# caburu/gym-supplychain

Measured on AMD Instinct MI355X. Metric: env-steps/sec at 65536 envs/GPU, beergame-v0; 1/2/4/8 MI355X, higher is better.
Workload: dtype int32; 1 GPU; beergame-v0 step() x 65536 envs/GPU (BASELINE configs[1]; configs[4] at N=8); n_envs_per_gpu=65536, levels=4, weeks=35, auto_reset=True, ledgers=True, orders_history=True, episode_return_allgather=False, parallelism=env-shard x1

## Files before the change

gym-supplychain_amd/csrc/scg_beergame.hip:

```cpp

#include <cstdarg>
#include <cstdio>
#include <ctime>
#include <vector>

#include "scg_beergame_kernels.h"

namespace scg {

__global__ __launch_bounds__(kBlock) void poisson_demand_kernel(const BgArgs a, int32_t weeks,
                                                                int32_t* __restrict__ out) {
  const int64_t n = static_cast<int64_t>(blockIdx.x) * kBlock + threadIdx.x;
  if (n >= a.n) return;
  for (int32_t w = 1; w <= weeks; ++w) out[(int64_t)(w - 1) * a.n + n] = week_demand(a, n, w, a.episode);
}

__global__ __launch_bounds__(kBlock) void uniform_ints_kernel(uint32_t k0, uint32_t k1, int64_t env_offset,
                                                              int64_t n_envs, int32_t rows, int32_t width,
                                                              uint32_t tag, int32_t lo, uint32_t range,
                                                              int32_t* __restrict__ out) {
  const int64_t n = static_cast<int64_t>(blockIdx.x) * kBlock + threadIdx.x;
  if (n >= n_envs) return;
  const uint32_t env = static_cast<uint32_t>(env_offset + n);
  const int32_t words = rows * width;
  for (int32_t j0 = 0; j0 < words; j0 += 4) {
    const scg::U4 r = scg::philox4x32_10(scg::U4{env, tag, static_cast<uint32_t>(j0 >> 2), SCG_STREAM_ACTION}, k0, k1);
    const uint32_t w4[4] = {r.x, r.y, r.z, r.w};
#pragma unroll
    for (int s = 0; s < 4; ++s) {
      const int32_t j = j0 + s;
      if (j < words) {
        const uint32_t v = static_cast<uint32_t>((static_cast<uint64_t>(w4[s]) * range) >> 32);
        const int32_t rrow = j / width, col = j - rrow * width;
        out[((int64_t)rrow * n_envs + n) * width + col] = lo + static_cast<int32_t>(v);
      }
    }
  }
}

int launch_reset(int L, dim3 grid, hipStream_t s, const BgArgs& a) {
  switch (L) {
#define X(l) case l: return bg_launch_reset<l>(grid, s, a);
    SCG_LEVEL_CASES(X)
#undef X
    default: return fail(SCG_ERR_INVALID, "levels=%d outside 1..%d", L, SCG_BG_MAX_LEVELS);
  }
}

int launch_step2(int L, dim3 grid, hipStream_t s, const BgArgs& a, const WeekInfo& wk) {
  switch (L) {
#define X(l) case l: return bg_launch_step2<l>(grid, s, a, wk);
    SCG_LEVEL_CASES(X)
#undef X
    default: return fail(SCG_ERR_INVALID, "levels=%d outside 1..%d", L, SCG_BG_MAX_LEVELS);
// ... 8 lines not shown
#undef X
    default: return fail(SCG_ERR_INVALID, "levels=%d outside 1..%d", L, SCG_BG_MAX_LEVELS);
  }
}

int launch_server(int L, int demand_mode, hipStream_t s, scg_bg_server_box* box, uint32_t exit_seen,
                  uint32_t idle_ticks) {
  switch (L) {
#define X(l) case l: return bg_launch_server<l>(s, demand_mode, box, exit_seen, idle_ticks);
    SCG_LEVEL_CASES(X)
#undef X
    default: return fail(SCG_ERR_INVALID, "levels=%d outside 1..%d", L, SCG_BG_MAX_LEVELS);
  }
}

int launch_slab(int demand_mode, int L, dim3 grid, hipStream_t s, int32_t* slab, const int32_t* act, int32_t* out,
                uint32_t n32, uint32_t wpack, uint32_t week, uint32_t episode, uint32_t k0, uint32_t k1,
                const BgSlabArgs& a, hipEvent_t ev0, hipEvent_t ev1) {
  switch (L) {
#define X(l) case l: return bg_launch_slab<l>(demand_mode, grid, s, slab, act, out, n32, wpack, week, episode, k0, k1, a, ev0, ev1);
    SCG_LEVEL_CASES(X)
#undef X
    default: return fail(SCG_ERR_INVALID, "levels=%d outside 1..%d", L, SCG_BG_MAX_LEVELS);
  }
}

int launch_rollout(int L, dim3 grid, hipStream_t s, const BgArgs& a, int32_t K, const RolloutWeeks& weeks,
                   const int32_t* acts, int32_t* obs, int32_t* rew) {
  switch (L) {
#define X(l) case l: return bg_launch_rollout<l>(grid, s, a, K, weeks, acts, obs, rew);
    SCG_LEVEL_CASES(X)
#undef X
    default: return fail(SCG_ERR_INVALID, "levels=%d outside 1..%d", L, SCG_BG_MAX_LEVELS);
  }
}
// ... 2 lines not shown
  const int64_t NL = N * L;
  if (NL % 4 != 0) return fail(SCG_ERR_INVALID, "slab layout needs n_envs * levels %% 4 == 0 (got %lld)", (long long)NL);
  if (R < 1 || R > 127) return fail(SCG_ERR_INVALID, "slab layout needs 1 <= ring_slots <= 127");
  off[SCG_SLAB_ERROR] = 0;
  for (int f = 0; f < 6; ++f) off[SCG_SLAB_INVENTORY + f] = kSlabHeader + f * NL;
  off[SCG_SLAB_RING] = kSlabHeader + 6 * NL;
  off[SCG_SLAB_EPISODE_RETURN] = kSlabHeader + (6 + R) * NL;
  off[SCG_SLAB_FINAL_RETURN] = off[SCG_SLAB_EPISODE_RETURN] + 2 * N;
  off[SCG_SLAB_HISTORY] = off[SCG_SLAB_FINAL_RETURN] + 2 * N;
  off[SCG_SLAB_TOTAL] = off[SCG_SLAB_HISTORY] + (history ? static_cast<int64_t>(T + 1) * NL : 0);
  return SCG_OK;
}

bool slab_ready(const scg_bg_config* cfg, const scg_bg_state* st, const int32_t* obs, const int32_t* reward,
                const int32_t* terminal_obs) {
  if (!st->slab || cfg->variant != 1) return false;
  int64_t off[SCG_SLAB_FIELDS];
  const bool hist = st->orders_history != nullptr;
  if (slab_layout(cfg->levels, st->n_envs, cfg->ring_slots, cfg->max_weeks, hist, off) != SCG_OK) return false;
  int32_t* b = st->slab;
  const bool ledgers = st->inventory_costs != nullptr, returns = st->episode_return != nullptr;
  return st->inventory == b + off[SCG_SLAB_INVENTORY] && st->backlog == b + off[SCG_SLAB_BACKLOG] &&
         st->orders_placed == b + off[SCG_SLAB_ORDERS] && st->shipments == b + off[SCG_SLAB_RING] &&
         (!ledgers || (st->inventory_costs == b + off[SCG_SLAB_INV_COSTS] &&
                       st->backlog_costs == b + off[SCG_SLAB_BACKLOG_COSTS])) &&
         ledgers == (st->backlog_costs != nullptr) &&
         (!returns || (reinterpret_cast<int32_t*>(st->episode_return) == b + off[SCG_SLAB_EPISODE_RETURN] &&
                       reinterpret_cast<int32_t*>(st->final_return) == b + off[SCG_SLAB_FINAL_RETURN])) &&
         (!hist || st->orders_history == b + off[SCG_SLAB_HISTORY]) &&
         st->error_flags == b + off[SCG_SLAB_ERROR] && reward == obs + st->n_envs * cfg->levels &&
         (!terminal_obs || terminal_obs == b + off[SCG_SLAB_TERMINAL_OBS]);
// ... 55 lines not shown
  a.guard = week_guard(cfg->levels, cfg->inv_cost, cfg->backlog_cost);
  a.err_host = st->error_host;
  if (cfg->variant == 2) {
    a.pen_acc = st->penalty_costs;
    a.max_stock = cfg->max_stock;
    a.penalty = cfg->exceeded_capacity_penalty;
    a.stochastic_delays = cfg->stochastic_delays;
    a.delay_lo = cfg->delay_lo;
    a.delay_hi = cfg->delay_hi;
  }
  return a;
}

inline dim3 grid_for(int64_t n) { return dim3(static_cast<unsigned>((n + kBlock - 1) / kBlock)); }

}

using namespace scg;

extern "C" {

int scg_bg_struct_sizes(size_t* config_size, size_t* state_size) {
  if (config_size) *config_size = sizeof(scg_bg_config);
  if (state_size) *state_size = sizeof(scg_bg_state);
  return SCG_OK;
}

int scg_poisson_table(double lam, uint32_t* out, int32_t cap) {
  if (!(lam >= 0.0) || std::isinf(lam)) return -fail(SCG_ERR_INVALID, "poisson lambda must be finite and >= 0");
  if (!out || cap <= 0) return -fail(SCG_ERR_INVALID, "null/empty threshold buffer");
// ... 112 lines not shown

int scg_bg_step(const scg_bg_config* cfg, scg_bg_state* st, const int32_t* action, int32_t* obs,
                int32_t* reward, int32_t* terminal_obs, uint32_t flags, int32_t* done, void* stream) {
  return scg_bg_step_timed(cfg, st, action, obs, reward, terminal_obs, flags, done, nullptr, nullptr, stream);
}

int scg_bg_step_timed(const scg_bg_config* cfg, scg_bg_state* st, const int32_t* action, int32_t* obs,
                      int32_t* reward, int32_t* terminal_obs, uint32_t flags, int32_t* done, void* start_event,
                      void* stop_event, void* stream) {
  if (int rc = check_state(cfg, st)) return rc;
  if (!action || !obs || !reward) return fail(SCG_ERR_INVALID, "action/obs/reward buffers are required");
  if (int rc = check_step(cfg, st)) return rc;
  const int32_t w = st->week + 1;
  const WeekInfo wk = week_info(cfg, w, flags);
  if (slab_ready(cfg, st, obs, reward, terminal_obs)) {
    BgSlabArgs sa;
    std::memset(&sa, 0, sizeof(sa));
    sa.pthr = cfg->poisson_thresholds;
    sa.demand_table = cfg->demand_table;
    sa.pthr_len = cfg->poisson_len;
    sa.h = cfg->inv_cost;
    sa.b = cfg->backlog_cost;
    sa.demand_fixed = wk.demand_fixed;
    sa.demand_lo = cfg->demand_lo;
    sa.demand_hi = cfg->demand_hi;
    sa.ship_value = cfg->initial_shipment_value;
    sa.orders_value = cfg->initial_orders_value;
    sa.init_slots = init_slots(cfg);
    sa.env_offset = st->env_offset;
    sa.guard = week_guard(cfg->levels, cfg->inv_cost, cfg->backlog_cost);
    sa.err_host = st->error_host;
    for (int l = 0; l < cfg->levels; ++l) sa.init_inv[l] = cfg->initial_inventory[l];
    uint32_t wpack = pack_week_slab(wk);
    wpack |= (wk.flags & 1) ? SW_TERMINAL : 0u;
    wpack |= (wk.flags & 2) ? SW_AUTORESET : 0u;
    wpack |= st->inventory_costs ? SW_LEDGERS : 0u;
    wpack |= st->episode_return ? SW_RETURNS : 0u;
    wpack |= st->orders_history ? SW_HISTORY : 0u;
    wpack |= static_cast<uint32_t>(cfg->ring_slots) << 24;
    if (int rc = launch_slab(cfg->demand_mode, cfg->levels, grid_for(st->n_envs), static_cast<hipStream_t>(stream),
                             st->slab, action, obs, static_cast<uint32_t>(st->n_envs), wpack, static_cast<uint32_t>(w),
                             st->episode, static_cast<uint32_t>(st->seed & 0xffffffffu),
                             static_cast<uint32_t>(st->seed >> 32), sa, static_cast<hipEvent_t>(start_event),
                             static_cast<hipEvent_t>(stop_event)))
      return rc;
    if (wk.flags & 2) {
      st->week = 0;
      st->episode += 1;
    } else {
      st->week = w;
    }
    if (done) *done = (wk.flags & 1) ? 1 : 0;
    return SCG_OK;
  }
  BgArgs a = make_args(cfg, st);
  a.act = action;
  a.obs = obs;
  a.rew = reward;
  a.term_obs = terminal_obs;
// ... 280 lines not shown
```

gym-supplychain_amd/csrc/scg_beergame_kernels.h:

```cpp
#pragma once

#include <hip/hip_ext.h>
#include <hip/hip_runtime.h>

#include <algorithm>
#include <cmath>
#include <cstdint>
#include <cstdlib>
#include <cstring>

#include "scg_common.h"
#include "scg_mailbox.h"
#include "scg_const.h"
#include "scg_philox.h"
#include "scgpu.h"

namespace scg {

enum : int32_t { MODE_DIRECT = 0, MODE_STORE = 1, MODE_ADD = 2, MODE_DROP = 3 };
constexpr int32_t PLAN_ARRIVE = 4;
inline int32_t plan_mode(int32_t p) { return p & 3; }
inline bool plan_arrive(int32_t p) { return (p & PLAN_ARRIVE) != 0; }
inline int32_t plan_delay(int32_t p) { return (p >> 8) & 0xff; }

// ... 79 lines not shown
    for (int c = 0; c < L / 4; ++c)
      reinterpret_cast<int4*>(p)[c] = make_int4(v[4 * c], v[4 * c + 1], v[4 * c + 2], v[4 * c + 3]);
  } else if constexpr (L % 2 == 0) {
#pragma unroll
    for (int c = 0; c < L / 2; ++c) reinterpret_cast<int2*>(p)[c] = make_int2(v[2 * c], v[2 * c + 1]);
  } else {
#pragma unroll
    for (int l = 0; l < L; ++l) p[l] = v[l];
  }
}

#ifndef SCG_BG_STORE
#define SCG_BG_STORE 1
#endif
typedef int v4i32 __attribute__((ext_vector_type(4)));

template <int L>
__device__ __forceinline__ void store_row_p(int32_t* __restrict__ p, const int32_t (&v)[L]) {
  if constexpr (SCG_BG_STORE != 0 && L % 4 == 0) {
#pragma unroll
    for (int c = 0; c < L / 4; ++c) {
      const v4i32 x = {v[4 * c], v[4 * c + 1], v[4 * c + 2], v[4 * c + 3]};
      if constexpr (SCG_BG_STORE == 1) {
        __builtin_nontemporal_store(x, reinterpret_cast<v4i32*>(p) + c);
      } else {
        asm volatile("global_store_dwordx4 %0, %1, off sc1\n\ts_nop 1" ::"v"(reinterpret_cast<v4i32*>(p) + c), "v"(x)
                     : "memory");
      }
    }
  } else {
// ... 8 lines not shown
  for (int l = 0; l < L; ++l) v[l] = x;
  store_row_p<L>(p, v);
}

template <int L>
__device__ __forceinline__ void fill_row(int32_t* __restrict__ p, int32_t x) {
  int32_t v[L];
#pragma unroll
  for (int l = 0; l < L; ++l) v[l] = x;
  store_row<L>(p, v);
}

__device__ __forceinline__ int32_t poisson_count_scalar(ConstTab<uint32_t> thr, int32_t len, uint32_t u) {
  int32_t x = 0;
  int k = 0;
  for (; k + 8 <= len; k += 8) {
#pragma unroll
    for (int j = 0; j < 8; ++j) x += (thr[k + j] <= u) ? 1 : 0;
  }
  for (; k < len; ++k) x += (thr[k] <= u) ? 1 : 0;
  return x;
}

__device__ __forceinline__ int32_t poisson_invert(const BgArgs& a, uint32_t u) {
  return poisson_count_scalar(const_tab(a.pthr), a.pthr_len, u);
}

template <int DM = -1>
__device__ __forceinline__ int32_t week_demand(const BgArgs& a, int64_t n, int32_t week,
                                               uint32_t episode) {
// ... 371 lines not shown
      __syncthreads();
      served = true;
    }
    if (ex != exit_seen) break;
    if (served) {
      t0 = __builtin_amdgcn_s_memrealtime();
      continue;
    }
    if (__builtin_amdgcn_s_memrealtime() - t0 > idle_ticks) break;
    __builtin_amdgcn_s_sleep(2);
  }
  __builtin_amdgcn_fence(__ATOMIC_RELEASE, "");
  if (lane == 0) __hip_atomic_store(&box->exit_seq, ex, __ATOMIC_RELEASE, __HIP_MEMORY_SCOPE_SYSTEM);
}

struct BgSlabArgs {
  const uint32_t* pthr;
  const int32_t* demand_table;
  int32_t pthr_len;
  int32_t h, b;
  int32_t demand_fixed;
  int32_t demand_lo, demand_hi;
  int32_t ship_value, orders_value, init_slots;
  int64_t env_offset;
  int32_t guard;
  int32_t* err_host;
  int32_t init_inv[SCG_BG_MAX_LEVELS];
};


constexpr uint32_t SW_TERMINAL = 1u << 18, SW_AUTORESET = 1u << 19, SW_LEDGERS = 1u << 20, SW_RETURNS = 1u << 21,
                   SW_HISTORY = 1u << 22;
constexpr int kSlabHeader = 4;

template <int L, int DM>
__global__ __launch_bounds__(kBlock) void bg_step_slab_kernel(int32_t* __restrict__ slab, const int32_t* __restrict__ act_p,
                                                              int32_t* __restrict__ out, uint32_t n32, uint32_t wpack,
                                                              uint32_t week, uint32_t episode, uint32_t key0,
                                                              uint32_t key1, const BgSlabArgs a) {
  const int64_t n = static_cast<int64_t>(blockIdx.x) * kBlock + threadIdx.x;
  if (n >= static_cast<int64_t>(n32)) return;
  const int32_t read_slot = static_cast<int32_t>(wpack & 0xffu) - 1;
  const int32_t write_slot = static_cast<int32_t>((wpack >> 8) & 0xffu);
  const int32_t mode = static_cast<int32_t>((wpack >> 16) & 3u);
  const int32_t R = static_cast<int32_t>((wpack >> 24) & 0x7fu);
  const bool terminal = wpack & SW_TERMINAL, autoreset = wpack & SW_AUTORESET;
  const bool ledgers = wpack & SW_LEDGERS, returns = wpack & SW_RETURNS, history = wpack & SW_HISTORY;
  const int64_t NL = static_cast<int64_t>(n32) * L;
  const int64_t row = n * L;
  int32_t* const rows = slab + kSlabHeader;
  int32_t* const inv_p = rows, *const bk_p = rows + NL, *const op_p = rows + 2 * NL;
  int32_t* const iacc_p = rows + 3 * NL, *const bacc_p = rows + 4 * NL, *const term_p = rows + 5 * NL;
  int32_t* const ring_p = rows + 6 * NL;
  int64_t* const ret_p = reinterpret_cast<int64_t*>(rows + (6 + R) * NL);
  int64_t* const fret_p = ret_p + n32;
  int32_t* const hist_p = reinterpret_cast<int32_t*>(fret_p + n32);
// ... 2 lines not shown
  zero_row<L>(due);
  zero_row<L>(cur);
  zero_row<L>(iacc);
  zero_row<L>(bacc);
  load_row<L>(inv_p + row, inv);
  load_row<L>(bk_p + row, bk);
  load_row<L>(op_p + row, op);
  load_row<L>(act_p + row, act);
  if (read_slot >= 0) load_row<L>(ring_p + read_slot * NL + row, due);
  if (mode == MODE_ADD) load_row<L>(ring_p + write_slot * NL + row, cur);
  if (ledgers && !autoreset) {
    load_row<L>(iacc_p + row, iacc);
    load_row<L>(bacc_p + row, bacc);
  }
  const int64_t ret0 = returns ? ret_p[n] : 0;
  export_error(n, terminal, slab, a.err_host);
  int32_t demand;
  if constexpr (DM == SCG_DEMAND_FIXED) {
    demand = a.demand_fixed;
  } else if constexpr (DM == SCG_DEMAND_TABLE) {
    demand = a.demand_table[static_cast<int64_t>(week - 1) * n32 + n];
  } else if constexpr (DM == SCG_DEMAND_UNIFORM) {
    const uint32_t w = scg::philox_word(key0, key1, static_cast<uint32_t>(a.env_offset + n), episode, week - 1,
                                        SCG_STREAM_BG2_DEMAND);
    demand = a.demand_lo + static_cast<int32_t>((static_cast<uint64_t>(w) * static_cast<uint32_t>(a.demand_hi - a.demand_lo)) >> 32);
  } else {
    const uint32_t u = scg::philox_word(key0, key1, static_cast<uint32_t>(a.env_offset + n), episode, week - 1,
                                        SCG_STREAM_DEMAND);
    demand = poisson_count_scalar(const_tab(a.pthr), a.pthr_len, u);
  }

  int32_t ship[L], obs[L];
  bool ovf = false;
  const int32_t reward = week_update<L>(a.h, a.b, a.guard, demand, mode == MODE_DIRECT, due, inv, bk, op, act, ship,
                                        obs, cur, iacc, bacc, ovf);
  if (mode == MODE_STORE) {
    store_row_p<L>(ring_p + write_slot * NL + row, ship);
  } else if (mode == MODE_ADD) {
    store_row_p<L>(ring_p + write_slot * NL + row, cur);
  }
  out[NL + n] = reward;
  if (history) store_row_p<L>(hist_p + static_cast<int64_t>(week) * NL + row, op);
  const int64_t ret = ret0 + reward;
  if (terminal) {
    store_row_p<L>(term_p + row, obs);
    if (returns) fret_p[n] = ret;
  }
  if (autoreset) {
    int32_t v[L];
#pragma unroll
    for (int l = 0; l < L; ++l) v[l] = a.init_inv[l];
    store_row_p<L>(inv_p + row, v);
    store_row_p<L>(out + row, v);
    fill_row_p<L>(bk_p + row, 0);
    fill_row_p<L>(op_p + row, a.orders_value);
    for (int t = 1; t <= a.init_slots; ++t) fill_row_p<L>(ring_p + (t % R) * NL + row, a.ship_value);
    if (ledgers) {
      fill_row_p<L>(iacc_p + row, 0);
      fill_row_p<L>(bacc_p + row, 0);
    }
    if (history) fill_row_p<L>(hist_p + row, a.orders_value);
    if (returns) ret_p[n] = 0;
    note_overflow(slab, ovf);
    return;
  }
  store_row_p<L>(inv_p + row, inv);
  store_row_p<L>(bk_p + row, bk);
  store_row_p<L>(op_p + row, op);
  store_row_p<L>(out + row, obs);
  if (ledgers) {
    store_row_p<L>(iacc_p + row, iacc);
    store_row_p<L>(bacc_p + row, bacc);
  }
  if (returns) ret_p[n] = ret;
  note_overflow(slab, ovf);
}
// ... 235 lines not shown
    hbm.load(s, v);
    lds.store(s, v);
  }
  rollout_body<L>(a, n, K, weeks, acts, obs_out, rew_out, lds);
  for (int s = 0; s < a.ring_slots; ++s) {
    int32_t v[L];
    lds.load(s, v);
    hbm.store(s, v);
  }
}

#ifndef SCG_MODULE_LAUNCH
#define SCG_MODULE_LAUNCH 1
#endif

template <int L, int DM>
int launch_slab_module(dim3 grid, hipStream_t s, int32_t* slab, const int32_t* act, int32_t* out, uint32_t n32,
                       uint32_t wpack, uint32_t week, uint32_t episode, uint32_t k0, uint32_t k1, const BgSlabArgs& a) {
  static hipFunction_t fn = nullptr;
  if (!fn && hipGetFuncBySymbol(&fn, reinterpret_cast<const void*>(&bg_step_slab_kernel<L, DM>)) != hipSuccess)
    return fail(SCG_ERR_HIP, "hipGetFuncBySymbol(bg_step_slab_kernel) failed");
  BgSlabArgs args = a;
  void* params[] = {&slab, &act, &out, &n32, &wpack, &week, &episode, &k0, &k1, &args};
  if (hipModuleLaunchKernel(fn, grid.x, 1, 1, kBlock, 1, 1, 0, s, params, nullptr) != hipSuccess)
    return fail(SCG_ERR_HIP, "hipModuleLaunchKernel(bg_step_slab_kernel) failed");
  return SCG_OK;
}

template <int L>
int bg_launch_reset(dim3 grid, hipStream_t s, const BgArgs& a) {
  hipLaunchKernelGGL(bg_reset_kernel<L>, grid, dim3(kBlock), 0, s, a);
  return check_launch("bg_reset_kernel");
}

template <int L>
int bg_launch_step2(dim3 grid, hipStream_t s, const BgArgs& a, const WeekInfo& wk) {
  hipLaunchKernelGGL(bg2_step_kernel<L>, grid, dim3(kBlock), 0, s, a, wk);
  return check_launch("bg2_step_kernel");
// ... 27 lines not shown
      hipLaunchKernelGGL(HIP_KERNEL_NAME(bg_server_kernel<L, SCG_DEMAND_TABLE>), dim3(1), dim3(kServerBlock), 0, s, box,
                         exit_seen, idle_ticks);
      break;
    case SCG_DEMAND_UNIFORM:
      hipLaunchKernelGGL(HIP_KERNEL_NAME(bg_server_kernel<L, SCG_DEMAND_UNIFORM>), dim3(1), dim3(kServerBlock), 0, s, box,
                         exit_seen, idle_ticks);
      break;
    default:
      hipLaunchKernelGGL(HIP_KERNEL_NAME(bg_server_kernel<L, SCG_DEMAND_POISSON>), dim3(1), dim3(kServerBlock), 0, s, box,
                         exit_seen, idle_ticks);
  }
  return check_launch("bg_server_kernel");
}

template <int L, int DM>
int bg_launch_slab_dm(dim3 grid, hipStream_t s, int32_t* slab, const int32_t* act, int32_t* out, uint32_t n32,
                      uint32_t wpack, uint32_t week, uint32_t episode, uint32_t k0, uint32_t k1, const BgSlabArgs& a,
                      hipEvent_t ev0, hipEvent_t ev1) {
  if (ev0 || ev1) {
    hipExtLaunchKernelGGL(HIP_KERNEL_NAME(bg_step_slab_kernel<L, DM>), grid, dim3(kBlock), 0, s, ev0, ev1, 0, slab, act,
                          out, n32, wpack, week, episode, k0, k1, a);
    return check_launch("bg_step_slab_kernel");
  }
  if (SCG_MODULE_LAUNCH) return launch_slab_module<L, DM>(grid, s, slab, act, out, n32, wpack, week, episode, k0, k1, a);
  hipLaunchKernelGGL(HIP_KERNEL_NAME(bg_step_slab_kernel<L, DM>), grid, dim3(kBlock), 0, s, slab, act, out, n32, wpack,
                     week, episode, k0, k1, a);
  return check_launch("bg_step_slab_kernel");
}

template <int L>
int bg_launch_slab(int demand_mode, dim3 grid, hipStream_t s, int32_t* slab, const int32_t* act, int32_t* out,
                   uint32_t n32, uint32_t wpack, uint32_t week, uint32_t episode, uint32_t k0, uint32_t k1,
                   const BgSlabArgs& a, hipEvent_t ev0, hipEvent_t ev1) {
  switch (demand_mode) {
    case SCG_DEMAND_FIXED:
      return bg_launch_slab_dm<L, SCG_DEMAND_FIXED>(grid, s, slab, act, out, n32, wpack, week, episode, k0, k1, a, ev0, ev1);
    case SCG_DEMAND_TABLE:
      return bg_launch_slab_dm<L, SCG_DEMAND_TABLE>(grid, s, slab, act, out, n32, wpack, week, episode, k0, k1, a, ev0, ev1);
    case SCG_DEMAND_UNIFORM:
      return bg_launch_slab_dm<L, SCG_DEMAND_UNIFORM>(grid, s, slab, act, out, n32, wpack, week, episode, k0, k1, a, ev0,
                                                      ev1);
    default:
      return bg_launch_slab_dm<L, SCG_DEMAND_POISSON>(grid, s, slab, act, out, n32, wpack, week, episode, k0, k1, a, ev0,
                                                      ev1);
  }
}

template <int L>
int bg_launch_rollout(dim3 grid, hipStream_t s, const BgArgs& a, int32_t K, const RolloutWeeks& weeks,
                      const int32_t* acts, int32_t* obs, int32_t* rew) {
  const size_t lds = static_cast<size_t>(a.ring_slots) * L * kBlock * sizeof(int32_t);
  if (lds <= 64 * 1024) {
    hipLaunchKernelGGL(bg_rollout_lds_kernel<L>, grid, dim3(kBlock), lds, s, a, K, weeks, acts, obs, rew);
    return check_launch("bg_rollout_lds_kernel");
  }
  hipLaunchKernelGGL(bg_rollout_kernel<L>, grid, dim3(kBlock), 0, s, a, K, weeks, acts, obs, rew);
  return check_launch("bg_rollout_kernel");
}

#define SCG_LEVEL_CASES(X) X(1) X(2) X(3) X(4) X(5) X(6) X(7) X(8) X(9) X(10) X(11) X(12) X(13) X(14) X(15) X(16)

#define SCG_BG_LAUNCHERS(EXT, l)                                                                                     \
  EXT template int bg_launch_reset<l>(dim3, hipStream_t, const BgArgs&);                                            \
  EXT template int bg_launch_step2<l>(dim3, hipStream_t, const BgArgs&, const WeekInfo&);                           \
  EXT template int bg_launch_step<l>(dim3, hipStream_t, const BgArgs&, const WeekInfo&, hipEvent_t, hipEvent_t);    \
  EXT template int bg_launch_server<l>(hipStream_t, int, scg_bg_server_box*, uint32_t, uint32_t);                   \
  EXT template int bg_launch_slab<l>(int, dim3, hipStream_t, int32_t*, const int32_t*, int32_t*, uint32_t, uint32_t, \
                                     uint32_t, uint32_t, uint32_t, uint32_t, const BgSlabArgs&, hipEvent_t,         \
                                     hipEvent_t);                                                                    \
  EXT template int bg_launch_rollout<l>(dim3, hipStream_t, const BgArgs&, int32_t, const RolloutWeeks&,             \
                                        const int32_t*, int32_t*, int32_t*);
#define SCG_BG_EXTERN_LEVEL(l) SCG_BG_LAUNCHERS(extern, l)
SCG_LEVEL_CASES(SCG_BG_EXTERN_LEVEL)
#undef SCG_BG_EXTERN_LEVEL

}
```

gym-supplychain_amd/gym_supplychain_amd/_native.py:

```python
import ctypes
import os

import torch

LIB_NAME = "libscgpu.so"
LIB_PATH = os.path.join(os.path.dirname(os.path.abspath(__file__)), LIB_NAME)
ABI_VERSION = 7

SCG_OK = 0
SCG_ERR_INVALID = 1
SCG_ERR_PAST_HORIZON = 2
SCG_ERR_NOT_RESET = 3
SCG_ERR_HIP = 4
SCG_PENDING = 5

SCG_DEMAND_FIXED = 0
SCG_DEMAND_TABLE = 1
SCG_DEMAND_POISSON = 2
SCG_DEMAND_UNIFORM = 3

SCG_BG_AUTORESET = 1
SCG_SC_SERIAL = 2
SCG_STREAM_DEMAND = 0
SCG_STREAM_ACTION = 1
# ... 48 lines not shown
        ("episode", ctypes.c_uint32),
        ("week", ctypes.c_int32),
        ("inventory", ctypes.c_void_p),
        ("backlog", ctypes.c_void_p),
        ("orders_placed", ctypes.c_void_p),
        ("shipments", ctypes.c_void_p),
        ("inventory_costs", ctypes.c_void_p),
        ("backlog_costs", ctypes.c_void_p),
        ("orders_history", ctypes.c_void_p),
        ("episode_return", ctypes.c_void_p),
        ("final_return", ctypes.c_void_p),
        ("penalty_costs", ctypes.c_void_p),
        ("error_flags", ctypes.c_void_p),
        ("error_host", ctypes.c_void_p),
        ("slab", ctypes.c_void_p),
    ]


BG_SERVER_SLOTS = 15
BG_SERVER_ARGS_BYTES = 512


class BgServerLine(ctypes.Structure):
    _fields_ = [("req_seq", ctypes.c_uint32), ("cmd", ctypes.c_int32), ("wpack", ctypes.c_uint32),
                ("week", ctypes.c_int32), ("demand_fixed", ctypes.c_int32), ("n_inline", ctypes.c_int32),
                ("gen", ctypes.c_uint32), ("check", ctypes.c_uint32), ("action", ctypes.c_int32 * 8)]


class BgServerBox(ctypes.Structure):
    _fields_ = [("req", BgServerLine * (BG_SERVER_SLOTS + 1)), ("done_seq", ctypes.c_uint32 * 16),
                ("n_slots", ctypes.c_uint32), ("exit_req", ctypes.c_uint32), ("exit_seq", ctypes.c_uint32),
# ... 347 lines not shown
```

gym-supplychain_amd/gym_supplychain_amd/envs/beergame_env.py:

```python
import atexit
import ctypes
import numbers
import os
import weakref

import numpy as np
import torch

from .. import _native as nat
from .. import checkpoint as ckpt
from .. import spaces
from . import resident
from ..distributed import entropy_seed

STD_LEVELS = 4
STD_DEMAND = [4] * 4 + [8] * 31
STD_INVENTORY = 12
STD_SHIP_DELAY = 2
STD_SHIP_VALUE = 4
STD_ORDERS_VALUE = 4
STD_INV_COST = 1
STD_BACKLOG_COST = 2

_I32 = (-(2 ** 31), 2 ** 31 - 1)
# ... 119 lines not shown
                raise ValueError(f"demand table must be int32 [{T}, {n_envs}] on {dev}")
            self._table = table.contiguous()
            c.demand_table = self._table.data_ptr()
        if mode == nat.SCG_DEMAND_POISSON:
            thr = nat.poisson_table(poisson_lambda)
            self.poisson_lambda = float(poisson_lambda)
            self._thresholds = torch.tensor(np.asarray(thr, dtype=np.uint32).view(np.int32), **i32)
            c.poisson_thresholds = self._thresholds.data_ptr()
            c.poisson_len = len(thr)
        nat.check(nat.lib.scg_bg_prepare(ctypes.byref(c)))
        self._cfg = c
        self.ring_slots = R = c.ring_slots

        v2 = c.variant == 2
        off = (ctypes.c_int64 * nat.SLAB_FIELDS)()
        self._slab = None
        if state_slab and nat.lib.scg_bg_slab_layout(ctypes.byref(c), n_envs, int(bool(track_history)), off) == 0:
            self._slab = torch.zeros(off[nat.SLAB_TOTAL], **i32)

            def rows(field, k=1):
                return self._slab[off[field]: off[field] + k * n_envs * L].view(*((k,) if k > 1 else ()), n_envs, L)

            def i64(field):
                return self._slab[off[field]: off[field] + 2 * n_envs].view(torch.int64)

            self._err = self._slab[off[nat.SLAB_ERROR]: off[nat.SLAB_ERROR] + 1]
            self._inv, self._bk, self._op = rows(nat.SLAB_INVENTORY), rows(nat.SLAB_BACKLOG), rows(nat.SLAB_ORDERS)
            self._ring = rows(nat.SLAB_RING, R) if R > 1 else rows(nat.SLAB_RING).unsqueeze(0)
            self._inv_costs = rows(nat.SLAB_INV_COSTS) if track_costs else None
            self._bk_costs = rows(nat.SLAB_BACKLOG_COSTS) if track_costs else None
            self._hist = rows(nat.SLAB_HISTORY, T + 1) if track_history else None
            self._ret = i64(nat.SLAB_EPISODE_RETURN) if track_returns else None
            self._final_ret = i64(nat.SLAB_FINAL_RETURN) if track_returns else None
# ... 20 lines not shown

        s = nat.BgState()
        s.n_envs, s.env_offset, s.seed = n_envs, int(env_offset), int(seed) & 0xFFFFFFFFFFFFFFFF
        s.episode, s.week = 0, -1
        s.inventory, s.backlog, s.orders_placed = self._inv.data_ptr(), self._bk.data_ptr(), self._op.data_ptr()
        s.shipments = self._ring.data_ptr()
        s.inventory_costs = self._inv_costs.data_ptr() if track_costs else None
        s.backlog_costs = self._bk_costs.data_ptr() if track_costs else None
        s.orders_history = self._hist.data_ptr() if track_history else None
        s.episode_return = self._ret.data_ptr() if track_returns else None
        s.final_return = self._final_ret.data_ptr() if track_returns else None
        s.penalty_costs = self._pen_costs.data_ptr() if self._pen_costs is not None else None
        s.error_flags = self._err.data_ptr()
        s.error_host = self._err_word.dev
        s.slab = self._slab.data_ptr() if self._slab is not None else None
        self._st = s
        self._cfg_ref = ctypes.byref(self._cfg)
        self._st_ref = ctypes.byref(self._st)
        self._done_flag = ctypes.c_int32(0)
        self._done_ref = ctypes.byref(self._done_flag)
        self._flags = nat.SCG_BG_AUTORESET if self.auto_reset else 0
        self._act_shape = (n_envs, L)
        self._obs_ptr, self._rew_ptr = self._obs.data_ptr(), self._rew.data_ptr()
        self._term_ptr = self._term_obs.data_ptr()
        self._cfg_addr, self._st_addr = ctypes.addressof(self._cfg), ctypes.addressof(self._st)
        self._fast_step, self._fast_step_timed = nat.fast.bg_step, nat.fast.bg_step_timed
        self._step_args = nat.BgStepArgs(self._cfg_addr, self._st_addr, self._obs_ptr, self._rew_ptr, self._term_ptr,
                                         self._flags)
        self._step_handle = ctypes.addressof(self._step_args)
        self._fast_step_h = nat.fast.bg_step_h
# ... 603 lines not shown
```

include/scgpu.h:

```cpp
#ifndef SCGPU_H
#define SCGPU_H

#include <stddef.h>
#include <stdint.h>

#ifdef __cplusplus
extern "C" {
#endif

#define SCG_ABI_VERSION 7

#if defined(__GNUC__)
#define SCG_API __attribute__((visibility("default")))
#else
#define SCG_API
#endif

#define SCG_BG_MAX_LEVELS 16
#define SCG_BG_MAX_WEEKS 4096
#define SCG_BG_MAX_DELAY 4096
#define SCG_POISSON_MAX 256
#define SCG_BG_ROLLOUT_MAX 128

typedef enum scg_status {
  SCG_OK = 0,
// ... 50 lines not shown
  uint32_t episode;
  int32_t week;
  int32_t* inventory;
  int32_t* backlog;
  int32_t* orders_placed;
  int32_t* shipments;
  int32_t* inventory_costs;
  int32_t* backlog_costs;
  int32_t* orders_history;
  int64_t* episode_return;
  int64_t* final_return;
  int32_t* penalty_costs;
  int32_t* error_flags;
  int32_t* error_host;
  int32_t* slab;
} scg_bg_state;

enum scg_bg_slab_field {
  SCG_SLAB_ERROR = 0,
  SCG_SLAB_INVENTORY,
  SCG_SLAB_BACKLOG,
  SCG_SLAB_ORDERS,
  SCG_SLAB_INV_COSTS,
  SCG_SLAB_BACKLOG_COSTS,
  SCG_SLAB_TERMINAL_OBS,
  SCG_SLAB_RING,
  SCG_SLAB_EPISODE_RETURN,
  SCG_SLAB_FINAL_RETURN,
  SCG_SLAB_HISTORY,
  SCG_SLAB_TOTAL,
  SCG_SLAB_FIELDS
// ... 271 lines not shown
```

Before: 13.22 billion env-steps/s.

## Move slab step constants into a device-resident block and shrink kernel arguments

The per-step constants (costs, guard, demand bounds, init values, pointers) move out of the by-value kernel argument struct into a 64-byte-aligned device buffer. A tiny kernel fills it only when a hash of the config changes. The step kernel now takes a small argument list and loads the constants with scalar loads. Poisson thresholds are also cached as a padded 40-entry table read as vector scalar loads. This cuts kernel argument marshalling and host packing per step, at the cost of an ABI change, an extra state field, and hash-based invalidation that could miss a change to the table contents behind the same pointer.

```diff
diff --git a/gym-supplychain_amd/csrc/scg_beergame.hip b/gym-supplychain_amd/csrc/scg_beergame.hip
--- a/gym-supplychain_amd/csrc/scg_beergame.hip
+++ b/gym-supplychain_amd/csrc/scg_beergame.hip
@@ -38,6 +38,26 @@
   }
 }
 
+__global__ __launch_bounds__(64) void bg_slab_consts_kernel(BgSlabConst* __restrict__ dst, const BgSlabConst v) {
+  const int q = threadIdx.x;
+  if (q < kFastThr) dst->thr[q] = (v.pthr && q < v.pthr_len) ? v.pthr[q] : 0xffffffffu;
+  if (q < SCG_BG_MAX_LEVELS) dst->init_inv[q] = v.init_inv[q];
+  if (q != 63) return;
+  dst->env_base = v.env_base;
+  dst->pthr_len = v.pthr_len;
+  dst->h = v.h;
+  dst->b = v.b;
+  dst->guard = v.guard;
+  dst->demand_lo = v.demand_lo;
+  dst->demand_hi = v.demand_hi;
+  dst->ship_value = v.ship_value;
+  dst->orders_value = v.orders_value;
+  dst->init_slots = v.init_slots;
+  dst->err_host = v.err_host;
+  dst->demand_table = v.demand_table;
+  dst->pthr = v.pthr;
+}
+
 int launch_reset(int L, dim3 grid, hipStream_t s, const BgArgs& a) {
   switch (L) {
 #define X(l) case l: return bg_launch_reset<l>(grid, s, a);
@@ -76,11 +96,10 @@
   }
 }
 
-int launch_slab(int demand_mode, int L, dim3 grid, hipStream_t s, int32_t* slab, const int32_t* act, int32_t* out,
-                uint32_t n32, uint32_t wpack, uint32_t week, uint32_t episode, uint32_t k0, uint32_t k1,
-                const BgSlabArgs& a, hipEvent_t ev0, hipEvent_t ev1) {
+int launch_slab(int demand_mode, int L, dim3 grid, hipStream_t s, const SlabLaunch& a, hipEvent_t ev0,
+                hipEvent_t ev1) {
   switch (L) {
-#define X(l) case l: return bg_launch_slab<l>(demand_mode, grid, s, slab, act, out, n32, wpack, week, episode, k0, k1, a, ev0, ev1);
+#define X(l) case l: return bg_launch_slab<l>(demand_mode, grid, s, a, ev0, ev1);
     SCG_LEVEL_CASES(X)
 #undef X
     default: return fail(SCG_ERR_INVALID, "levels=%d outside 1..%d", L, SCG_BG_MAX_LEVELS);
@@ -113,7 +132,7 @@
 
 bool slab_ready(const scg_bg_config* cfg, const scg_bg_state* st, const int32_t* obs, const int32_t* reward,
                 const int32_t* terminal_obs) {
-  if (!st->slab || cfg->variant != 1) return false;
+  if (!st->slab || !st->step_consts || cfg->variant != 1) return false;
   int64_t off[SCG_SLAB_FIELDS];
   const bool hist = st->orders_history != nullptr;
   if (slab_layout(cfg->levels, st->n_envs, cfg->ring_slots, cfg->max_weeks, hist, off) != SCG_OK) return false;
@@ -199,6 +218,50 @@
 
 inline dim3 grid_for(int64_t n) { return dim3(static_cast<unsigned>((n + kBlock - 1) / kBlock)); }
 
+BgSlabConst slab_consts(const scg_bg_config* cfg, const scg_bg_state* st) {
+  BgSlabConst v;
+  std::memset(&v, 0, sizeof(v));
+  v.env_base = static_cast<uint32_t>(st->env_offset);
+  v.pthr_len = cfg->demand_mode == SCG_DEMAND_POISSON ? cfg->poisson_len : 0;
+  v.h = cfg->inv_cost;
+  v.b = cfg->backlog_cost;
+  v.guard = week_guard(cfg->levels, cfg->inv_cost, cfg->backlog_cost);
+  v.demand_lo = cfg->demand_lo;
+  v.demand_hi = cfg->demand_hi;
+  v.ship_value = cfg->initial_shipment_value;
+  v.orders_value = cfg->initial_orders_value;
+  v.init_slots = init_slots(cfg);
+  v.err_host = st->error_host;
+  v.demand_table = cfg->demand_table;
+  v.pthr = cfg->demand_mode == SCG_DEMAND_POISSON ? cfg->poisson_thresholds : nullptr;
+  for (int l = 0; l < cfg->levels; ++l) v.init_inv[l] = cfg->initial_inventory[l];
+  return v;
+}
+
+uint64_t slab_consts_tag(const BgSlabConst& v, const void* block) {
+  static_assert(offsetof(BgSlabConst, thr) % 8 == 0, "hashed as 64-bit words");
+  uint64_t w[offsetof(BgSlabConst, thr) / 8];
+  std::memcpy(w, &v, sizeof(w));
+  uint64_t h = 0x9E3779B97F4A7C15ull ^ reinterpret_cast<uintptr_t>(block);
+  for (uint64_t x : w) {
+    h = (h ^ x) * 0xFF51AFD7ED558CCDull;
+    h ^= h >> 29;
+  }
+  return h | 1u;
+}
+
+int sync_slab_consts(const scg_bg_config* cfg, scg_bg_state* st, hipStream_t s) {
+  const BgSlabConst v = slab_consts(cfg, st);
+  const uint64_t tag = slab_consts_tag(v, st->step_consts);
+  if (tag == st->step_consts_tag) return SCG_OK;
+  if (reinterpret_cast<uintptr_t>(st->step_consts) % alignof(BgSlabConst) != 0)
+    return fail(SCG_ERR_INVALID, "step_consts must be %d-byte aligned", static_cast<int>(alignof(BgSlabConst)));
+  hipLaunchKernelGGL(bg_slab_consts_kernel, dim3(1), dim3(64), 0, s, static_cast<BgSlabConst*>(st->step_consts), v);
+  if (int rc = check_launch("bg_slab_consts_kernel")) return rc;
+  st->step_consts_tag = tag;
+  return SCG_OK;
+}
+
 }
 
 using namespace scg;
@@ -341,23 +404,7 @@
   const int32_t w = st->week + 1;
   const WeekInfo wk = week_info(cfg, w, flags);
   if (slab_ready(cfg, st, obs, reward, terminal_obs)) {
-    BgSlabArgs sa;
-    std::memset(&sa, 0, sizeof(sa));
-    sa.pthr = cfg->poisson_thresholds;
-    sa.demand_table = cfg->demand_table;
-    sa.pthr_len = cfg->poisson_len;
-    sa.h = cfg->inv_cost;
-    sa.b = cfg->backlog_cost;
-    sa.demand_fixed = wk.demand_fixed;
-    sa.demand_lo = cfg->demand_lo;
-    sa.demand_hi = cfg->demand_hi;
-    sa.ship_value = cfg->initial_shipment_value;
-    sa.orders_value = cfg->initial_orders_value;
-    sa.init_slots = init_slots(cfg);
-    sa.env_offset = st->env_offset;
-    sa.guard = week_guard(cfg->levels, cfg->inv_cost, cfg->backlog_cost);
-    sa.err_host = st->error_host;
-    for (int l = 0; l < cfg->levels; ++l) sa.init_inv[l] = cfg->initial_inventory[l];
+    if (int rc = sync_slab_consts(cfg, st, static_cast<hipStream_t>(stream))) return rc;
     uint32_t wpack = pack_week_slab(wk);
     wpack |= (wk.flags & 1) ? SW_TERMINAL : 0u;
     wpack |= (wk.flags & 2) ? SW_AUTORESET : 0u;
@@ -365,11 +412,11 @@
     wpack |= st->episode_return ? SW_RETURNS : 0u;
     wpack |= st->orders_history ? SW_HISTORY : 0u;
     wpack |= static_cast<uint32_t>(cfg->ring_slots) << 24;
-    if (int rc = launch_slab(cfg->demand_mode, cfg->levels, grid_for(st->n_envs), static_cast<hipStream_t>(stream),
-                             st->slab, action, obs, static_cast<uint32_t>(st->n_envs), wpack, static_cast<uint32_t>(w),
-                             st->episode, static_cast<uint32_t>(st->seed & 0xffffffffu),
-                             static_cast<uint32_t>(st->seed >> 32), sa, static_cast<hipEvent_t>(start_event),
-                             static_cast<hipEvent_t>(stop_event)))
+    const SlabLaunch sl{st->slab, action, obs, static_cast<const BgSlabConst*>(st->step_consts), st->seed,
+                        static_cast<uint32_t>(st->n_envs), wpack, static_cast<uint32_t>(w), st->episode,
+                        wk.demand_fixed};
+    if (int rc = launch_slab(cfg->demand_mode, cfg->levels, grid_for(st->n_envs), static_cast<hipStream_t>(stream), sl,
+                             static_cast<hipEvent_t>(start_event), static_cast<hipEvent_t>(stop_event)))
       return rc;
     if (wk.flags & 2) {
       st->week = 0;
diff --git a/gym-supplychain_amd/csrc/scg_beergame_kernels.h b/gym-supplychain_amd/csrc/scg_beergame_kernels.h
--- a/gym-supplychain_amd/csrc/scg_beergame_kernels.h
+++ b/gym-supplychain_amd/csrc/scg_beergame_kernels.h
@@ -117,6 +117,8 @@
 #define SCG_BG_STORE 1
 #endif
 typedef int v4i32 __attribute__((ext_vector_type(4)));
+typedef uint32_t u32x8 __attribute__((ext_vector_type(8)));
+typedef uint32_t u32x16 __attribute__((ext_vector_type(16)));
 
 template <int L>
 __device__ __forceinline__ void store_row_p(int32_t* __restrict__ p, const int32_t (&v)[L]) {
@@ -155,6 +157,22 @@
 __device__ __forceinline__ int32_t poisson_count_scalar(ConstTab<uint32_t> thr, int32_t len, uint32_t u) {
   int32_t x = 0;
   int k = 0;
+  for (; k + 8 <= len; k += 8) {
+#pragma unroll
+    for (int j = 0; j < 8; ++j) x += (thr[k + j] <= u) ? 1 : 0;
+  }
+  for (; k < len; ++k) x += (thr[k] <= u) ? 1 : 0;
+  return x;
+}
+
+constexpr int kFastThr = 40;
+__host__ __device__ __forceinline__ int32_t poisson_count_padded(const uint32_t (&fast)[kFastThr],
+                                                                 ConstTab<uint32_t> thr, int32_t len, uint32_t u) {
+  int32_t x = 0;
+#pragma unroll
+  for (int q = 0; q < kFastThr; ++q) x += (fast[q] <= u) ? 1 : 0;
+  x = x < len ? x : len;
+  int k = kFastThr;
   for (; k + 8 <= len; k += 8) {
 #pragma unroll
     for (int j = 0; j < 8; ++j) x += (thr[k + j] <= u) ? 1 : 0;
@@ -556,20 +574,21 @@
   if (lane == 0) __hip_atomic_store(&box->exit_seq, ex, __ATOMIC_RELEASE, __HIP_MEMORY_SCOPE_SYSTEM);
 }
 
-struct BgSlabArgs {
-  const uint32_t* pthr;
-  const int32_t* demand_table;
+struct alignas(64) BgSlabConst {
+  uint32_t env_base;
   int32_t pthr_len;
-  int32_t h, b;
-  int32_t demand_fixed;
+  int32_t h, b, guard;
   int32_t demand_lo, demand_hi;
   int32_t ship_value, orders_value, init_slots;
-  int64_t env_offset;
-  int32_t guard;
   int32_t* err_host;
+  const int32_t* demand_table;
+  const uint32_t* pthr;
   int32_t init_inv[SCG_BG_MAX_LEVELS];
+  uint32_t thr[kFastThr];
 };
-
+static_assert(sizeof(BgSlabConst) <= SCG_BG_STEP_CONSTS_BYTES && offsetof(BgSlabConst, err_host) == 40 &&
+                  offsetof(BgSlabConst, init_inv) == 64 && offsetof(BgSlabConst, thr) == 128,
+              "BgSlabConst layout");
 
 constexpr uint32_t SW_TERMINAL = 1u << 18, SW_AUTORESET = 1u << 19, SW_LEDGERS = 1u << 20, SW_RETURNS = 1u << 21,
                    SW_HISTORY = 1u << 22;
@@ -577,11 +596,14 @@
 
 template <int L, int DM>
 __global__ __launch_bounds__(kBlock) void bg_step_slab_kernel(int32_t* __restrict__ slab, const int32_t* __restrict__ act_p,
-                                                              int32_t* __restrict__ out, uint32_t n32, uint32_t wpack,
-                                                              uint32_t week, uint32_t episode, uint32_t key0,
-                                                              uint32_t key1, const BgSlabArgs a) {
+                                                              int32_t* __restrict__ out,
+                                                              const BgSlabConst* __restrict__ consts, uint64_t key,
+                                                              uint32_t n32, uint32_t wpack, uint32_t week,
+                                                              uint32_t episode, int32_t demand_fixed) {
   const int64_t n = static_cast<int64_t>(blockIdx.x) * kBlock + threadIdx.x;
   if (n >= static_cast<int64_t>(n32)) return;
+  const ConstTab<BgSlabConst> c = const_tab(consts);
+  const uint32_t key0 = static_cast<uint32_t>(key), key1 = static_cast<uint32_t>(key >> 32);
   const int32_t read_slot = static_cast<int32_t>(wpack & 0xffu) - 1;
   const int32_t write_slot = static_cast<int32_t>((wpack >> 8) & 0xffu);
   const int32_t mode = static_cast<int32_t>((wpack >> 16) & 3u);
@@ -614,25 +636,47 @@
     load_row<L>(bacc_p + row, bacc);
   }
   const int64_t ret0 = returns ? ret_p[n] : 0;
-  export_error(n, terminal, slab, a.err_host);
+  const int32_t h = c->h, b = c->b, guard = c->guard;
+  int32_t* const err_host = c->err_host;
   int32_t demand;
   if constexpr (DM == SCG_DEMAND_FIXED) {
-    demand = a.demand_fixed;
+    demand = demand_fixed;
+    asm volatile("" : "+s"(demand) : "s"(h), "s"(b), "s"(guard), "s"(err_host));
   } else if constexpr (DM == SCG_DEMAND_TABLE) {
-    demand = a.demand_table[static_cast<int64_t>(week - 1) * n32 + n];
+    const int32_t* table = c->demand_table;
+    asm volatile("" : "+s"(table) : "s"(h), "s"(b), "s"(guard), "s"(err_host));
+    demand = table[static_cast<int64_t>(week - 1) * n32 + n];
   } else if constexpr (DM == SCG_DEMAND_UNIFORM) {
-    const uint32_t w = scg::philox_word(key0, key1, static_cast<uint32_t>(a.env_offset + n), episode, week - 1,
+    const int32_t lo = c->demand_lo, hi = c->demand_hi;
+    uint32_t env_base = c->env_base;
+    asm volatile("" : "+s"(env_base) : "s"(lo), "s"(hi), "s"(h), "s"(b), "s"(guard), "s"(err_host));
+    const uint32_t w = scg::philox_word(key0, key1, env_base + static_cast<uint32_t>(n), episode, week - 1,
                                         SCG_STREAM_BG2_DEMAND);
-    demand = a.demand_lo + static_cast<int32_t>((static_cast<uint64_t>(w) * static_cast<uint32_t>(a.demand_hi - a.demand_lo)) >> 32);
+    demand = lo + static_cast<int32_t>((static_cast<uint64_t>(w) * static_cast<uint32_t>(hi - lo)) >> 32);
   } else {
-    const uint32_t u = scg::philox_word(key0, key1, static_cast<uint32_t>(a.env_offset + n), episode, week - 1,
+    static_assert(kFastThr == 40, "the thresholds are read as 16 + 16 + 8 dwords");
+    const u32x16 t0 = *reinterpret_cast<ConstTab<u32x16>>(c->thr);
+    const u32x16 t1 = *reinterpret_cast<ConstTab<u32x16>>(c->thr + 16);
+    const u32x8 t2 = *reinterpret_cast<ConstTab<u32x8>>(c->thr + 32);
+    const int32_t len = c->pthr_len;
+    const ConstTab<uint32_t> pthr = const_tab(c->pthr);
+    uint32_t env_base = c->env_base;
+    asm volatile("" : "+s"(env_base) : "s"(t0), "s"(t1), "s"(t2), "s"(len), "s"(pthr), "s"(h), "s"(b), "s"(guard),
+                 "s"(err_host));
+    uint32_t fast[kFastThr];
+#pragma unroll
+    for (int q = 0; q < 16; ++q) fast[q] = t0[q], fast[16 + q] = t1[q];
+#pragma unroll
+    for (int q = 0; q < 8; ++q) fast[32 + q] = t2[q];
+    const uint32_t u = scg::philox_word(key0, key1, env_base + static_cast<uint32_t>(n), episode, week - 1,
                                         SCG_STREAM_DEMAND);
-    demand = poisson_count_scalar(const_tab(a.pthr), a.pthr_len, u);
-  }
+    demand = poisson_count_padded(fast, pthr, len, u);
+  }
+  export_error(n, terminal, slab, err_host);
 
   int32_t ship[L], obs[L];
   bool ovf = false;
-  const int32_t reward = week_update<L>(a.h, a.b, a.guard, demand, mode == MODE_DIRECT, due, inv, bk, op, act, ship,
+  const int32_t reward = week_update<L>(h, b, guard, demand, mode == MODE_DIRECT, due, inv, bk, op, act, ship,
                                         obs, cur, iacc, bacc, ovf);
   if (mode == MODE_STORE) {
     store_row_p<L>(ring_p + write_slot * NL + row, ship);
@@ -649,17 +693,18 @@
   if (autoreset) {
     int32_t v[L];
 #pragma unroll
-    for (int l = 0; l < L; ++l) v[l] = a.init_inv[l];
+    for (int l = 0; l < L; ++l) v[l] = c->init_inv[l];
+    const int32_t orders_value = c->orders_value, ship_value = c->ship_value, init_slots = c->init_slots;
     store_row_p<L>(inv_p + row, v);
     store_row_p<L>(out + row, v);
     fill_row_p<L>(bk_p + row, 0);
-    fill_row_p<L>(op_p + row, a.orders_value);
-    for (int t = 1; t <= a.init_slots; ++t) fill_row_p<L>(ring_p + (t % R) * NL + row, a.ship_value);
+    fill_row_p<L>(op_p + row, orders_value);
+    for (int t = 1; t <= init_slots; ++t) fill_row_p<L>(ring_p + (t % R) * NL + row, ship_value);
     if (ledgers) {
       fill_row_p<L>(iacc_p + row, 0);
       fill_row_p<L>(bacc_p + row, 0);
     }
-    if (history) fill_row_p<L>(hist_p + row, a.orders_value);
+    if (history) fill_row_p<L>(hist_p + row, orders_value);
     if (returns) ret_p[n] = 0;
     note_overflow(slab, ovf);
     return;
@@ -925,14 +970,22 @@
 #define SCG_MODULE_LAUNCH 1
 #endif
 
+struct SlabLaunch {
+  int32_t* slab;
+  const int32_t* act;
+  int32_t* out;
+  const BgSlabConst* consts;
+  uint64_t key;
+  uint32_t n32, wpack, week, episode;
+  int32_t demand_fixed;
+};
+
 template <int L, int DM>
-int launch_slab_module(dim3 grid, hipStream_t s, int32_t* slab, const int32_t* act, int32_t* out, uint32_t n32,
-                       uint32_t wpack, uint32_t week, uint32_t episode, uint32_t k0, uint32_t k1, const BgSlabArgs& a) {
+int launch_slab_module(dim3 grid, hipStream_t s, SlabLaunch a) {
   static hipFunction_t fn = nullptr;
   if (!fn && hipGetFuncBySymbol(&fn, reinterpret_cast<const void*>(&bg_step_slab_kernel<L, DM>)) != hipSuccess)
     return fail(SCG_ERR_HIP, "hipGetFuncBySymbol(bg_step_slab_kernel) failed");
-  BgSlabArgs args = a;
-  void* params[] = {&slab, &act, &out, &n32, &wpack, &week, &episode, &k0, &k1, &args};
+  void* params[] = {&a.slab, &a.act, &a.out, &a.consts, &a.key, &a.n32, &a.wpack, &a.week, &a.episode, &a.demand_fixed};
   if (hipModuleLaunchKernel(fn, grid.x, 1, 1, kBlock, 1, 1, 0, s, params, nullptr) != hipSuccess)
     return fail(SCG_ERR_HIP, "hipModuleLaunchKernel(bg_step_slab_kernel) failed");
   return SCG_OK;
@@ -990,35 +1043,25 @@
 }
 
 template <int L, int DM>
-int bg_launch_slab_dm(dim3 grid, hipStream_t s, int32_t* slab, const int32_t* act, int32_t* out, uint32_t n32,
-                      uint32_t wpack, uint32_t week, uint32_t episode, uint32_t k0, uint32_t k1, const BgSlabArgs& a,
-                      hipEvent_t ev0, hipEvent_t ev1) {
+int bg_launch_slab_dm(dim3 grid, hipStream_t s, const SlabLaunch& a, hipEvent_t ev0, hipEvent_t ev1) {
   if (ev0 || ev1) {
-    hipExtLaunchKernelGGL(HIP_KERNEL_NAME(bg_step_slab_kernel<L, DM>), grid, dim3(kBlock), 0, s, ev0, ev1, 0, slab, act,
-                          out, n32, wpack, week, episode, k0, k1, a);
+    hipExtLaunchKernelGGL(HIP_KERNEL_NAME(bg_step_slab_kernel<L, DM>), grid, dim3(kBlock), 0, s, ev0, ev1, 0, a.slab,
+                          a.act, a.out, a.consts, a.key, a.n32, a.wpack, a.week, a.episode, a.demand_fixed);
     return check_launch("bg_step_slab_kernel");
   }
-  if (SCG_MODULE_LAUNCH) return launch_slab_module<L, DM>(grid, s, slab, act, out, n32, wpack, week, episode, k0, k1, a);
-  hipLaunchKernelGGL(HIP_KERNEL_NAME(bg_step_slab_kernel<L, DM>), grid, dim3(kBlock), 0, s, slab, act, out, n32, wpack,
-                     week, episode, k0, k1, a);
+  if (SCG_MODULE_LAUNCH) return launch_slab_module<L, DM>(grid, s, a);
+  hipLaunchKernelGGL(HIP_KERNEL_NAME(bg_step_slab_kernel<L, DM>), grid, dim3(kBlock), 0, s, a.slab, a.act, a.out,
+                     a.consts, a.key, a.n32, a.wpack, a.week, a.episode, a.demand_fixed);
   return check_launch("bg_step_slab_kernel");
 }
 
 template <int L>
-int bg_launch_slab(int demand_mode, dim3 grid, hipStream_t s, int32_t* slab, const int32_t* act, int32_t* out,
-                   uint32_t n32, uint32_t wpack, uint32_t week, uint32_t episode, uint32_t k0, uint32_t k1,
-                   const BgSlabArgs& a, hipEvent_t ev0, hipEvent_t ev1) {
+int bg_launch_slab(int demand_mode, dim3 grid, hipStream_t s, const SlabLaunch& a, hipEvent_t ev0, hipEvent_t ev1) {
   switch (demand_mode) {
-    case SCG_DEMAND_FIXED:
-      return bg_launch_slab_dm<L, SCG_DEMAND_FIXED>(grid, s, slab, act, out, n32, wpack, week, episode, k0, k1, a, ev0, ev1);
-    case SCG_DEMAND_TABLE:
-      return bg_launch_slab_dm<L, SCG_DEMAND_TABLE>(grid, s, slab, act, out, n32, wpack, week, episode, k0, k1, a, ev0, ev1);
-    case SCG_DEMAND_UNIFORM:
-      return bg_launch_slab_dm<L, SCG_DEMAND_UNIFORM>(grid, s, slab, act, out, n32, wpack, week, episode, k0, k1, a, ev0,
-                                                      ev1);
-    default:
-      return bg_launch_slab_dm<L, SCG_DEMAND_POISSON>(grid, s, slab, act, out, n32, wpack, week, episode, k0, k1, a, ev0,
-                                                      ev1);
+    case SCG_DEMAND_FIXED: return bg_launch_slab_dm<L, SCG_DEMAND_FIXED>(grid, s, a, ev0, ev1);
+    case SCG_DEMAND_TABLE: return bg_launch_slab_dm<L, SCG_DEMAND_TABLE>(grid, s, a, ev0, ev1);
+    case SCG_DEMAND_UNIFORM: return bg_launch_slab_dm<L, SCG_DEMAND_UNIFORM>(grid, s, a, ev0, ev1);
+    default: return bg_launch_slab_dm<L, SCG_DEMAND_POISSON>(grid, s, a, ev0, ev1);
   }
 }
 
@@ -1041,9 +1084,7 @@
   EXT template int bg_launch_step2<l>(dim3, hipStream_t, const BgArgs&, const WeekInfo&);                           \
   EXT template int bg_launch_step<l>(dim3, hipStream_t, const BgArgs&, const WeekInfo&, hipEvent_t, hipEvent_t);    \
   EXT template int bg_launch_server<l>(hipStream_t, int, scg_bg_server_box*, uint32_t, uint32_t);                   \
-  EXT template int bg_launch_slab<l>(int, dim3, hipStream_t, int32_t*, const int32_t*, int32_t*, uint32_t, uint32_t, \
-                                     uint32_t, uint32_t, uint32_t, uint32_t, const BgSlabArgs&, hipEvent_t,         \
-                                     hipEvent_t);                                                                    \
+  EXT template int bg_launch_slab<l>(int, dim3, hipStream_t, const SlabLaunch&, hipEvent_t, hipEvent_t);            \
   EXT template int bg_launch_rollout<l>(dim3, hipStream_t, const BgArgs&, int32_t, const RolloutWeeks&,             \
                                         const int32_t*, int32_t*, int32_t*);
 #define SCG_BG_EXTERN_LEVEL(l) SCG_BG_LAUNCHERS(extern, l)
diff --git a/gym-supplychain_amd/gym_supplychain_amd/_native.py b/gym-supplychain_amd/gym_supplychain_amd/_native.py
--- a/gym-supplychain_amd/gym_supplychain_amd/_native.py
+++ b/gym-supplychain_amd/gym_supplychain_amd/_native.py
@@ -5,7 +5,7 @@
 
 LIB_NAME = "libscgpu.so"
 LIB_PATH = os.path.join(os.path.dirname(os.path.abspath(__file__)), LIB_NAME)
-ABI_VERSION = 7
+ABI_VERSION = 8
 
 SCG_OK = 0
 SCG_ERR_INVALID = 1
@@ -86,7 +86,12 @@
         ("error_flags", ctypes.c_void_p),
         ("error_host", ctypes.c_void_p),
         ("slab", ctypes.c_void_p),
+        ("step_consts", ctypes.c_void_p),
+        ("step_consts_tag", ctypes.c_uint64),
     ]
+
+
+BG_STEP_CONSTS_BYTES = 512
 
 
 BG_SERVER_SLOTS = 15
diff --git a/gym-supplychain_amd/gym_supplychain_amd/envs/beergame_env.py b/gym-supplychain_amd/gym_supplychain_amd/envs/beergame_env.py
--- a/gym-supplychain_amd/gym_supplychain_amd/envs/beergame_env.py
+++ b/gym-supplychain_amd/gym_supplychain_amd/envs/beergame_env.py
@@ -157,9 +157,10 @@
 
         v2 = c.variant == 2
         off = (ctypes.c_int64 * nat.SLAB_FIELDS)()
-        self._slab = None
+        self._slab = self._step_consts = None
         if state_slab and nat.lib.scg_bg_slab_layout(ctypes.byref(c), n_envs, int(bool(track_history)), off) == 0:
             self._slab = torch.zeros(off[nat.SLAB_TOTAL], **i32)
+            self._step_consts = torch.zeros(nat.BG_STEP_CONSTS_BYTES // 4, **i32)
 
             def rows(field, k=1):
                 return self._slab[off[field]: off[field] + k * n_envs * L].view(*((k,) if k > 1 else ()), n_envs, L)
@@ -210,6 +211,8 @@
         s.error_flags = self._err.data_ptr()
         s.error_host = self._err_word.dev
         s.slab = self._slab.data_ptr() if self._slab is not None else None
+        s.step_consts = self._step_consts.data_ptr() if self._step_consts is not None else None
+        s.step_consts_tag = 0
         self._st = s
         self._cfg_ref = ctypes.byref(self._cfg)
         self._st_ref = ctypes.byref(self._st)
diff --git a/include/scgpu.h b/include/scgpu.h
--- a/include/scgpu.h
+++ b/include/scgpu.h
@@ -8,7 +8,7 @@
 extern "C" {
 #endif
 
-#define SCG_ABI_VERSION 7
+#define SCG_ABI_VERSION 8
 
 #if defined(__GNUC__)
 #define SCG_API __attribute__((visibility("default")))
@@ -89,7 +89,11 @@
   int32_t* error_flags;
   int32_t* error_host;
   int32_t* slab;
+  void* step_consts;
+  uint64_t step_consts_tag;
 } scg_bg_state;
+
+#define SCG_BG_STEP_CONSTS_BYTES 512
 
 enum scg_bg_slab_field {
   SCG_SLAB_ERROR = 0,
```

Measured after the change: 15.02 billion env-steps/s (median of 6 runs). 1.14x the previous value.
